# ami-iit/paper_gorbani_2025_humanoids_multi-rate-mpc-ironcub

Hardware: AMD Instinct MI355X
Metric: MPC solves/sec (whole node) + p50 single-solve latency, iRonCub paper horizon (higher is better)
Workload: dtype f64

## Files before the change

paper_gorbani_2025_humanoids_multi-rate-mpc-ironcub_amd/csrc/vsmpc_solve_body.inc:

```
#define VS_STAMP(i)                                                                        \
    do {                                                                                    \
        if constexpr (STAMPS) {                                                             \
            unsigned long long* st_ = late_args()->stamps;                                  \
            if (tid == 0 && st_ != nullptr) st_[size_t(blockIdx.x) * 16 + (i)] = __builtin_amdgcn_s_memtime(); \
        }                                                                                   \
    } while (0)
    unsigned long long t_acc[6] = {0, 0, 0, 0, 0, 0};
    unsigned long long t_mark = 0, stamp_t1 = 0, rt0 = 0;
    if constexpr (STAMPS) rt0 = __builtin_amdgcn_s_memrealtime();
#define VS_TIC()                                                     \
    do {                                                             \
        if constexpr (STAMPS) t_mark = __builtin_amdgcn_s_memtime(); \
    } while (0)
#define VS_TOC(i)                                                          \
    do {                                                                   \
        if constexpr (STAMPS) {                                            \
            const unsigned long long t_now = __builtin_amdgcn_s_memtime(); \
            t_acc[i] += t_now - t_mark;                                    \
            t_mark = t_now;                                                \
        }                                                                  \
    } while (0)
    using S = Smem<D, SMALL>;
    static_assert(!SMALL || (FORM == 1 && !TUNED), "the small-batch kind is the structured form of the shared kind");
    constexpr bool PIPE = FORM == 1;
    constexpr int QR_P0_STEPS = D::STRUCT_LONG ? 1 : 2;
    extern __shared__ __attribute__((aligned(16))) double smem[];
    double* sIn = smem + S::oIn;
    double* sA = smem + S::oA;
    double* sBj = smem + S::oBj;
    double* sBt = smem + S::oBt;
    double* sC = smem + S::oC;
    double* sVprev = smem + S::oVprev;
    double* sInvD = smem + S::oInvD;
    double* sW = smem + S::oW;
    double* sZ = smem + S::oZ;
    double* sSv = smem + S::oSv;
    double* sSvec = smem + S::oSvec;
    double* sV = smem + S::oV;
    double* sX = smem + S::oX;
    double* sF = smem + S::oF;
    double* sDt = smem + S::oDt;
    double* sCfg = smem + S::oCfg;
    int* sFlags = reinterpret_cast<int*>(smem + S::oFlags);
    double* sY = smem + S::oY;
    double* Lb = smem + S::oM;
    double* sXinv = smem + S::oXinv;
    double* sQP = smem + S::oQP;
    double* sU = smem + S::oU;

    const int inst = blockIdx.x;
    if (inst >= batch) return;
    int tid = threadIdx.x;
    int lane = tid & 63;
    const int wave = __builtin_amdgcn_readfirstlane(tid >> 6);
#define VS_REFRESH_IDS()                                                                     \
    do {                                                                                     \
        unsigned m_ = ~0u;                                                                   \
        asm volatile("" : "+s"(m_));                                                         \
        lane = int(__builtin_amdgcn_mbcnt_hi(m_, __builtin_amdgcn_mbcnt_lo(m_, 0u)));        \
        tid = (wave << 6) | lane;                                                            \
    } while (0)

    constexpr int TPW = TileTab<D, PIPE>::TPW;

    VS_STAMP(0);
    {
        static_assert(D::NIN % 2 == 0 && D::NVAR % 2 == 0 && D::NXS % 2 == 0 && D::NUO % 2 == 0, "double2 I/O");
        static_assert(D::NIN / 2 <= D::BLOCK, "one 16-byte load per thread covers the record");
        const double2* in2 = reinterpret_cast<const double2*>(in + size_t(inst) * D::NIN);
        double2* sIn2 = reinterpret_cast<double2*>(sIn);
        double2 rec = make_double2(0.0, 0.0);
        if (tid < D::NIN / 2) rec = in2[tid];
        constexpr int TUN0 = D::BLOCK - CFG_SIZE / 2;
        double2 trow = make_double2(0.0, 0.0);
        if constexpr (TUNED) {
            static_assert(CFG_SIZE == VSMPC_TUNE_SIZE && CFG_SIZE % 2 == 0 && CFG_VMAX == CFG_SIZE - 2, "row = sCfg + one pad");
            if (tid >= TUN0) trow = reinterpret_cast<const double2*>(tun + size_t(inst) * CFG_SIZE)[tid - TUN0];
        }
        if (tid < 4) sFlags[tid] = 0;
        if (tid < D::N) sDt[tid] = cfg.dt[tid];
        if constexpr (!TUNED) {
            if (tid >= 64 && tid < 64 + NWROWS) sCfg[CFG_SQ + tid - 64] = cfg.sq[tid - 64];
            if (tid >= 96 && tid < 96 + NJ) sCfg[CFG_WJ + tid - 96] = cfg.wj[tid - 96];
            if (tid == 128) {
                sCfg[CFG_WREG] = cfg.w_reg; sCfg[CFG_WTHR] = cfg.w_thr; sCfg[CFG_WINIT] = cfg.w_init;
                sCfg[CFG_VMIN] = cfg.vmin; sCfg[CFG_VMAX] = cfg.vmax;
            }
        }
        for (int i = tid; i < NX * NX + NX * NJ + NX * NTH + 28; i += D::BLOCK) sA[i] = 0.0;
        if (tid < D::NIN / 2) sIn2[tid] = rec;
        if constexpr (TUNED) {
            if (tid >= TUN0) {
                sCfg[2 * (tid - TUN0)] = trow.x;
                sCfg[2 * (tid - TUN0) + 1] = trow.y;
            }
            const bool fin = isfinite(trow.x) && (isfinite(trow.y) || tid == D::BLOCK - 1);
            __syncthreads();
            if (!fin) sFlags[0] = 1;
        } else {
            __syncthreads();
        }
    }
    p0_linearize<false, false, false>(cfg.use_jet, sIn, sA, sBj, sBt, sC, sVprev, tid, D::BLOCK);
    if (wave == 3) {
        if constexpr (FORM == 1) p0_joint_reduction<D, 0, QR_P0_STEPS>(smem, lane);
        else p0_joint_reduction<D>(smem, lane);
    }

    constexpr int NJROW = D::NV + NTH + 1, ZROW = D::NV + NTH;
    double* sJetT = sXinv;
    if constexpr (SMALL) sJetT = smem + S::oJetT;
    static_assert(SMALL || S::oJetT == S::oXinv, "the jet trajectories lie at the head of the X region");
    double* sGA = sJetT + NJROW * D::N;
    static_assert(D::NV + NTH <= 64 && (SMALL || NJROW * D::N + 6 * D::N <= S::NXT * D::TS), "jet trajectories fit the X region");
    if (wave == 1) {
        if (lane < D::NV + NTH) {
            const bool affl = lane >= D::NV;
            const int i = affl ? lane - D::NV : (lane & 3);
            const int blk = affl ? -1 : v_block_of_internal<D>(lane);
            const double jon = sA[(12 + i) * NX + 16 + i], ja = sA[(16 + i) * NX + 12 + i], jb = sA[(16 + i) * NX + 16 + i];
            const double c12 = sC[12 + i], c16 = sC[16 + i], b12 = sBt[(12 + i) * NTH + i], b16 = sBt[(16 + i) * NTH + i];
            const double t0 = sIn[VSMPC_IN_X0 + 12 + i], td0 = sIn[VSMPC_IN_X0 + 16 + i];
            const double bT = affl ? c12 : b12, bTd = affl ? c16 : b16;
            double T = affl ? t0 : 0.0, Td = affl ? td0 : 0.0;
#pragma unroll
            for (int k = 0; k < D::N; ++k) {
                sJetT[lane * D::N + k] = T;
                const double mT = (affl || throttle_block_of_stage<D>(k) == blk) ? 1.0 : 0.0;
                const double dT = fma(jon, Td, mT * bT);
                const double dTd = fma(ja, T, fma(jb, Td, mT * bTd));
                const double dt = sDt[k];
                T = fma(dt, dT, T);
                Td = fma(dt, dTd, Td);
            }
        }
        for (int k = lane; k < D::N; k += 64) sJetT[ZROW * D::N + k] = 0.0;
        if constexpr (FORM == 1) {
            const double am = sIn[VSMPC_IN_ALPHA] * sIn[VSMPC_IN_MASS];
            const double* R = sIn + VSMPC_IN_WRB;
            const double* gr = sIn + VSMPC_IN_GRAV;
            for (int e = lane; e < 6 * D::N; e += 64) {
                const int h = e / (3 * D::N), k = (e / 3) % D::N, r = e % 3;
                double g = 0.0;
#pragma unroll
                for (int c = 0; c < NTH; ++c) g = fma(sIn[VSMPC_IN_AMOM + (3 * h + r) * NTH + c], sJetT[(D::NV + c) * D::N + k], g);
                const double ch = h == 0 ? am * (R[0 + r] * gr[0] + R[3 + r] * gr[1] + R[6 + r] * gr[2]) : 0.0;
                sGA[e] = g + ch;
            }
        }
    }
    if constexpr (FORM == 1) {
        if (wave == 2) {
            for (int e = lane; e < S::sizeZero; e += 64) smem[S::oSZero + e] = 0.0;
            for (int e = lane; e < 12 * D::NREF; e += 64) {
                const int row = e % 12;
                const double off = row < 3 ? -sIn[VSMPC_IN_PREF + row] : ((row >= 6 && row < 9) ? -sIn[VSMPC_IN_RPYINIT + row - 6] : 0.0);
                smem[S::oSRefC + e] = sIn[VSMPC_IN_XREF + e] + off;
            }
        }
    }
    if constexpr (FORM == 1 && D::STRUCT_LONG) {
        for (int e = tid; e < S::sizeAc; e += D::BLOCK) smem[S::oSAc + e] = 0.0;
    }
    __syncthreads();
    if constexpr (FORM != 1) {
        for (int e = tid; e < 6 * D::N; e += D::BLOCK) {
            const int h = e / (3 * D::N), k = (e / 3) % D::N, r = e % 3, row = (h ? 9 : 3) + r;
            double g = 0.0;
#pragma unroll
            for (int c = 0; c < NTH; ++c) g = fma(sA[row * NX + 12 + c], sJetT[(D::NV + c) * D::N + k], g);
            sGA[e] = g;
        }
        __syncthreads();
    }

    VS_STAMP(1);
    VS_REFRESH_IDS();
    if constexpr (STAMPS) stamp_t1 = __builtin_amdgcn_s_memtime();
    d4 acc[TPW];
    if constexpr (FORM == 1) {
        static_assert(D::STRUCT_P1, "structured condensing is instantiated for horizons with Dims::STRUCT_P1");
        VS_TIC();
        if (wave < 2) {
            p1s_chain<D, 0, SMALL>(cfg, wave, lane, smem);
            if (wave == 0) p0_joint_reduction<D, QR_P0_STEPS, NJC>(smem, lane);
        } else {
            p1s_chain<D, 1, SMALL>(cfg, wave - 2, lane, smem);
        }
        VS_TOC(0);
        __syncthreads();
        VS_TOC(1);
        if constexpr (!D::STRUCT_LONG) {
            p1s_contract<D, SMALL>(smem, tid);
            __syncthreads();
        }
        VS_TOC(3);
        auto tail = [&](auto wcst) __attribute__((always_inline)) {
            constexpr int W = decltype(wcst)::value;
            if constexpr (SMALL) {
                static_for<0, TPW>([&](auto qcst) __attribute__((always_inline)) {
                    constexpr int q = decltype(qcst)::value;
                    if constexpr (small_instalment<D, TPW, W>(q) < 0) acc[q] = d4{0.0, 0.0, 0.0, 0.0};
                });
                const int ln0 = fresh_lane();
                small_form<D, TPW, W, 0>(sCfg, acc, Lb, smem + S::oQR + S::QR_GY, sVprev, ln0, (ln0 >> 4) * 17 + (ln0 & 15));
            } else {
                p1s_entries<D, TPW, W, PIPE>(acc, smem, lane);
            }
            VS_TOC(2);
            __syncthreads();
            VS_STAMP(2);
            constexpr TileTab<D, PIPE> tab{};
            double* dbgLw = nullptr;
            if constexpr (STAMPS && !SMALL) {
                double* dbgM = late_args()->dbgM;
                double* dbgL = late_args()->dbgL;
                dbgLw = dbgL != nullptr ? dbgL + size_t(inst) * D::NP * D::NP : nullptr;
                if (dbgM != nullptr) {
                    const int ln = fresh_lane();
                    static_for<0, TPW>([&](auto qcst) __attribute__((always_inline)) {
                        constexpr int q = decltype(qcst)::value;
                        constexpr int t = q * D::NWAVES + W;
                        if constexpr (tab.forms(t, W))
                            dump_hessian_tile<D>(dbgM + size_t(inst) * D::NP * D::NP, tab.ti[t], tab.tj[t], acc[q], sCfg,
                                                 smem + S::oQR + S::QR_GY, sVprev, ln);
                    });
                }
            }
            VS_STAMP(3);
            if constexpr (D::WG_PER_CU == 1) pin_tiles_agpr<TPW>(acc);
            const int ln = fresh_lane();
            cholesky_wave<D, TPW, W, STAMPS, PIPE, SMALL>(sCfg, acc, Lb, sInvD, smem + S::oQR + S::QR_GY, sVprev, sFlags, sXinv, sW, dbgLw, ln,
                                                  (ln >> 4) * 17 + (ln & 15), (ln & 15) * 17 + (ln >> 4), sZ);
            if constexpr (STAMPS) {
                if (dbgLw != nullptr) {
                    const int l2 = fresh_lane();
                    static_for<0, TPW>([&](auto qcst) __attribute__((always_inline)) {
                        constexpr int q = decltype(qcst)::value;
                        constexpr int t = q * D::NWAVES + W;
                        if constexpr (tab.holds(t, W) && tab.tj[t] < D::PVT && tab.ti[t] > tab.tj[t])
                            dump_factor_tile<D>(dbgLw, tab.ti[t], tab.tj[t], acc[q], l2);
                    });
                }
            }
        };
        switch (wave) {
            case 0: tail(std::integral_constant<int, 0>{}); break;
            case 1: tail(std::integral_constant<int, 1>{}); break;
            case 2: tail(std::integral_constant<int, 2>{}); break;
            default: tail(std::integral_constant<int, 3>{}); break;
        }
    } else {
#pragma unroll
        for (int q = 0; q < TPW; ++q) acc[q] = d4{0.0, 0.0, 0.0, 0.0};
        constexpr int CPT = D::CPT;
        const int pw = wave;
        const int ptid = tid;
        const int half = pw / (D::NWAVES / 2);
        const int xr0 = half ? 6 : 0, hr0 = half ? 9 : 3, er0 = half ? 23 : 20;
        const int yx0 = half ? 6 : 0, yh0 = half ? 9 : 3, ye0 = half ? 15 : 12;

        double M1[9], Sk[9], Ce[3], sqx[3], sqh[3], sqe[3];
        auto load_coeffs = [&]() __attribute__((always_inline)) {
#pragma unroll
            for (int r = 0; r < 3; ++r) {
#pragma unroll
                for (int c = 0; c < 3; ++c) {
                    M1[3 * r + c] = sA[(xr0 + r) * NX + hr0 + c];
                    Sk[3 * r + c] = sA[(hr0 + r) * NX + hr0 + c];
                }
                Ce[r] = sC[er0 + r];
                sqx[r] = sCfg[CFG_SQ + yx0 + r];
                sqh[r] = sCfg[CFG_SQ + yh0 + r];
                sqe[r] = sCfg[CFG_SQ + ye0 + r];
            }
        };
        const int ylane = (lane >> 4) * D::YS + (lane & 15);
        constexpr int NPASS = (D::N + 1) / 2;
        if constexpr (STAMPS) { t_mark = stamp_t1; VS_TOC(3); }

        int col[CPT], kind[CPT], blk[CPT];
        double aff[CPT], xs[CPT][3], hs[CPT][3], es[CPT][3], bha[CPT][3];
        const double* jetT[CPT];
        const double* gaT = sGA + half * 3 * D::N;
#pragma unroll
        for (int cc = 0; cc < CPT; ++cc) {
            const int c = cc * D::PCOLS + ptid % D::PCOLS;
            int comp = 0;
            col[cc] = c;
            kind[cc] = 3;
            blk[cc] = 0;
            if (c < D::NUY) { kind[cc] = 0; blk[cc] = c / NJC; comp = c - NJC * blk[cc]; }
            else if (c >= D::NU && c < D::NZ) { kind[cc] = 1; blk[cc] = v_block_of_internal<D>(c - D::NU); comp = (c - D::NU) & 3; }
            else if (c == D::NZ) { kind[cc] = 2; }
            const int jc = comp & 7, tc = comp & 3;
            const bool aff_col = kind[cc] == 2, jnt_col = kind[cc] == 0, thr_col = kind[cc] == 1;
            aff[cc] = aff_col ? 1.0 : 0.0;
#pragma unroll
            for (int r = 0; r < 3; ++r) {
                const double x0 = sIn[VSMPC_IN_X0 + xr0 + r], h0 = sIn[VSMPC_IN_X0 + hr0 + r], e0 = sIn[VSMPC_IN_X0 + er0 + r];
                const double bj = sBj[(hr0 + r) * NJ + jc], ch = sC[hr0 + r], at = sA[(hr0 + r) * NX + 12 + tc];
                xs[cc][r] = aff_col ? x0 : 0.0;
                hs[cc][r] = aff_col ? h0 : 0.0;
                es[cc][r] = aff_col ? e0 : 0.0;
                bha[cc][r] = jnt_col ? bj : (aff_col ? ch : (thr_col ? at : 0.0));
            }
            jetT[cc] = sJetT + (thr_col ? c - D::NU : ZROW) * D::N;
        }
        unsigned tpk[TilePack<D>::NWORDS];
#pragma unroll
        for (int k = 0; k < TilePack<D>::NWORDS; ++k) tpk[k] = kTilePack<D>.w[pw][k];
        const double* ybase = sY + ylane;
        constexpr bool UNROLLED = TPW <= SYRK_UNROLL_TPW;
        auto slot_word = [&](int q) __attribute__((always_inline)) {
            unsigned w = tpk[q >> 1];
            if constexpr (!UNROLLED) asm volatile("" : "+s"(w));
            return w;
        };
        auto slot_a = [&](int q) __attribute__((always_inline)) { return ybase + 16 * int((slot_word(q) >> (16 * (q & 1))) & 0xffu); };
        auto slot_b = [&](int q) __attribute__((always_inline)) { return ybase + 16 * int((slot_word(q) >> (16 * (q & 1) + 8)) & 0xffu); };
        auto rec_pass = [&](int m, int nnodes, double* sYm) __attribute__((always_inline)) {
            load_coeffs();
#pragma unroll
            for (int par = 0; par < 2; ++par) {
                if (par >= nnodes) break;
                const int k = 2 * m + par;
                const double dt = sDt[k];
                const int rc = k < D::NS ? 0 : k - D::NS;
                const double* xr = sIn + VSMPC_IN_XREF + rc * 12;
                double xrx[3], xrh[3], ga[3];
#pragma unroll
                for (int r = 0; r < 3; ++r) { xrx[r] = xr[yx0 + r]; xrh[r] = xr[yh0 + r]; ga[r] = gaT[3 * k + r]; }
#pragma unroll
                for (int cc = 0; cc < CPT; ++cc) {
                    const double tk = jetT[cc][k];
                    const bool actJ = (kind[cc] == 0 && joint_block_of_stage<D>(k) == blk[cc]) || kind[cc] == 2;
                    const double scale = kind[cc] == 1 ? tk : (actJ ? 1.0 : 0.0);
                    double dx[3], dh[3], de[3];
#pragma unroll
                    for (int r = 0; r < 3; ++r) {
                        double a0 = M1[3 * r] * hs[cc][0], a1 = scale * bha[cc][r], a2 = aff[cc] * ga[r];
#pragma unroll
                        for (int c = 1; c < 3; ++c) a0 = fma(M1[3 * r + c], hs[cc][c], a0);
#pragma unroll
                        for (int c = 0; c < 3; ++c) a1 = fma(Sk[3 * r + c], hs[cc][c], a1);
                        dx[r] = a0;
                        dh[r] = a1 + a2;
                        de[r] = fma(aff[cc], Ce[r], xs[cc][r]);
                    }
#pragma unroll
                    for (int r = 0; r < 3; ++r) { xs[cc][r] += dt * dx[r]; hs[cc][r] += dt * dh[r]; es[cc][r] += dt * de[r]; }
                    if (CPT == 1 || col[cc] < D::NP) {
                        double* Yn = sYm + 18 * par * D::YS + col[cc];
#pragma unroll
                        for (int r = 0; r < 3; ++r) {
                            const double vx = fma(-aff[cc], xrx[r], xs[cc][r]);
                            const double vh = fma(-aff[cc], xrh[r], hs[cc][r]);
                            Yn[(yx0 + r) * D::YS] = sqx[r] * vx;
                            Yn[(yh0 + r) * D::YS] = sqh[r] * vh;
                            Yn[(ye0 + r) * D::YS] = sqe[r] * es[cc][r];
                        }
                    }
                }
            }
            if (nnodes == 1)
                for (int i = ptid; i < 2 * D::YS; i += D::BLOCK) sYm[18 * D::YS + i] = 0.0;
        };
        auto syrk_fixed = [&](auto nks_c, auto nact_c) __attribute__((always_inline)) {
            constexpr int NKS = decltype(nks_c)::value, NACT = decltype(nact_c)::value;
            if constexpr (NACT > 0) {
                double ha[SYRK_DIST], hb[SYRK_DIST];
#pragma unroll
                for (int ks = 0; ks < SYRK_DIST; ++ks) {
                    ha[ks] = slot_a(NACT - 1)[ks * 4 * D::YS];
                    hb[ks] = slot_b(NACT - 1)[ks * 4 * D::YS];
                }
#pragma unroll
                for (int q = NACT - 1; q >= 0; --q) {
                    const int qn = q > 0 ? q - 1 : 0;
                    syrk_slot<D, NKS, true>(acc[q], slot_a(q), slot_b(q), ha, hb, slot_a(qn), slot_b(qn));
                }
            }
        };
        if constexpr (UNROLLED) {
            static_for<0, NPASS>([&](auto mc) __attribute__((always_inline)) {
                constexpr int m = decltype(mc)::value;
                constexpr int nnodes = (2 * m + 1 < D::N) ? 2 : 1;
                VS_TIC();
                rec_pass(m, nnodes, sY);
                VS_TOC(0);
                __syncthreads();
                VS_TOC(1);
                syrk_fixed(std::integral_constant<int, nnodes == 2 ? 9 : 5>{}, std::integral_constant<int, nact_max<D>(m)>{});
                VS_TOC(2);
                __syncthreads();
            });
        } else {
            static_for<0, PassGroups<D>::count()>([&](auto gc) __attribute__((always_inline)) {
                constexpr PassGroups<D> pg{};
                constexpr int g = decltype(gc)::value;
#pragma unroll 1
                for (int m = pg.start[g]; m < pg.end[g]; ++m) {
                    VS_TIC();
                    rec_pass(m, pg.nks[g] == 9 ? 2 : 1, sY);
                    VS_TOC(0);
                    __syncthreads();
                    VS_TOC(1);
                    syrk_fixed(std::integral_constant<int, pg.nks[g]>{}, std::integral_constant<int, pg.nact[g]>{});
                    VS_TOC(2);
                    __syncthreads();
                }
            });
        }
        VS_TIC();
    }
    VS_REFRESH_IDS();
    if constexpr (D::WG_PER_CU == 1) pin_tiles_agpr<TPW>(acc);

    static_assert(D::NWAVES == 4, "wave-specialised phases are instantiated for four wavefronts");
    constexpr int PVT = D::PVT;
    const int crow = (lane >> 4) * 17 + (lane & 15);
    const int lrow = (lane & 15) * 17 + (lane >> 4);
    double* dbgL = STAMPS ? late_args()->dbgL : nullptr;
    double* dbgLi = dbgL != nullptr ? dbgL + size_t(inst) * D::NP * D::NP : nullptr;
    VS_REFRESH_IDS();
    if constexpr (!PIPE) {
        int wave_c = wave;
        if constexpr (STAMPS) asm volatile("" : "+s"(wave_c));
        VS_STAMP(2);
        if constexpr (STAMPS) {
            const TileTab<D, PIPE>& tab = kTileTab<D, PIPE>;
            double* dbgM = late_args()->dbgM;
            if (dbgM != nullptr) {
#pragma unroll
                for (int q = 0; q < TPW; ++q) {
                    const int t = q * D::NWAVES + wave, tc = q * D::NWAVES + wave_c;
                    if (tab.forms(t, wave))
                        dump_hessian_tile<D>(dbgM + size_t(inst) * D::NP * D::NP, tab.ti[tc], tab.tj[tc], acc[q], sCfg,
                                             smem + S::oQR + S::QR_GY, sVprev, lane);
                }
            }
        }
        VS_STAMP(3);
        switch (wave) {
            case 0: cholesky_wave<D, TPW, 0, STAMPS, PIPE>(sCfg, acc, Lb, sInvD, smem + S::oQR + S::QR_GY, sVprev, sFlags, sXinv, sW, dbgLi, lane, crow, lrow, sZ); break;
            case 1: cholesky_wave<D, TPW, 1, STAMPS, PIPE>(sCfg, acc, Lb, sInvD, smem + S::oQR + S::QR_GY, sVprev, sFlags, sXinv, sW, dbgLi, lane, crow, lrow, sZ); break;
            case 2: cholesky_wave<D, TPW, 2, STAMPS, PIPE>(sCfg, acc, Lb, sInvD, smem + S::oQR + S::QR_GY, sVprev, sFlags, sXinv, sW, dbgLi, lane, crow, lrow, sZ); break;
            default: cholesky_wave<D, TPW, 3, STAMPS, PIPE>(sCfg, acc, Lb, sInvD, smem + S::oQR + S::QR_GY, sVprev, sFlags, sXinv, sW, dbgLi, lane, crow, lrow, sZ); break;
        }
        if constexpr (STAMPS) {
            const TileTab<D, PIPE>& tab = kTileTab<D, PIPE>;
            if (dbgLi != nullptr) {
#pragma unroll
                for (int q = 0; q < TPW; ++q) {
                    const int t = q * D::NWAVES + wave, tc = q * D::NWAVES + wave_c;
                    if (tab.holds(t, wave) && tab.tj[tc] < PVT && tab.ti[tc] > tab.tj[tc])
                        dump_factor_tile<D>(dbgLi, tab.ti[tc], tab.tj[tc], acc[q], lane);
                }
            }
        }
    }
    if (STAMPS && dbgLi != nullptr) {
        for (int e = tid; e < (D::NP - 16 * PVT) * (D::NP - 16 * PVT); e += D::BLOCK) {
            const int gr = 16 * PVT + e / (D::NP - 16 * PVT), gc = 16 * PVT + e % (D::NP - 16 * PVT);
            if (gc <= gr) dbgLi[size_t(gr) * D::NP + gc] = Lb[lower_at<D>(gr, gc)];
        }
    }

    VS_STAMP(4);
    VS_REFRESH_IDS();
    if constexpr (D::WG_PER_CU == 1) pin_tiles_agpr<TPW>(acc);
    const bool hold = sIn[VSMPC_IN_HOLD] != 0.0;
    constexpr int PV = D::PVT;
    auto init_corner_rhs = [&]() {
        if (tid >= 16 * PV && tid < D::NP) sW[tid] = tid < D::NZ ? -Lb[lower_at<D>(D::NZ, tid)] : 0.0;
    };
    init_corner_rhs();
    if (tid < D::NP) sZ[tid] = (hold && tid >= D::NZ - 4 && tid < D::NZ) ? sVprev[tid - (D::NZ - 4)] : 0.0;
    __syncthreads();

    auto corner_update = [&](int p) __attribute__((always_inline)) {
        if (p > PV) {
            if (tid >= 16 * PV && tid < 16 * p) {
                const double* T = Lb + tile_off<D>(p, tid >> 4) + (tid & 15);
                const double* zp = sZ + 16 * p;
                double a2 = 0.0;
#pragma unroll
                for (int k = 0; k < 16; ++k) a2 += T[k * 17] * zp[k];
                sW[tid] -= a2;
            }
            __syncthreads();
        }
    };
    auto sweep_tile = [&](int p, bool prescribed) {
        if (wave == 0) {
            const int j = lane & 15;
            const int gj = 16 * p + j;
            const double* Tpp = Lb + tile_off<D>(p, p) + j;
            double colv[16];
#pragma unroll
            for (int k = 0; k < 16; ++k) {
                const double t = Tpp[k * 17];
                colv[k] = k >= j ? t : 0.0;
            }
            double w = sW[gj];
            const bool fix = (gj >= D::NZ) || (gj >= D::NU && (prescribed || (hold && gj >= D::NZ - 4)));
            const double inv_eff = fix ? 0.0 : sInvD[gj];
            const double zadd = (fix && gj < D::NZ) ? sZ[gj] : 0.0;
            double z = 0.0;
#pragma unroll
            for (int k = 15; k >= 0; --k) {
                const double zk = readlane_f64(fma(w, inv_eff, zadd), k);
                z = (j == k) ? zk : z;
                w = fma(-colv[k], zk, w);
            }
            if (lane < 16) sZ[gj] = z;
        }
        __syncthreads();
        corner_update(p);
    };

    constexpr bool DUALQP = S::DUALQP;
    if constexpr (DUALQP) {
        constexpr int PL = D::NT - 1, KL = D::NZ - 16 * PL;
        static_assert(KL == D::NV - 16 && KL >= 4, "pins live in the last tile row");
        const double* X6 = sXinv + PV * D::TS;
        const double* L76 = Lb + tile_off<D>(PL, PV);
        const double* L77 = Lb + tile_off<D>(PL, PL);
        if (wave == 0) {
            const int j = lane & 15;
            const int gj = 16 * PL + j;
            const double* Tpp = L77 + j;
            double colv[KL], l76[KL], x6[16];
#pragma unroll
            for (int k = 0; k < KL; ++k) {
                const double t = Tpp[k * 17];
                colv[k] = k >= j ? t : 0.0;
                l76[k] = L76[k * 17 + j];
            }
#pragma unroll
            for (int i = 0; i < 16; ++i) x6[i] = X6[i * 17 + j];
            double w = sW[gj];
            double w6 = sW[16 * PV + j];
            const bool fix = (j >= KL) || (hold && j >= KL - 4);
            const double inv_eff = fix ? 0.0 : sInvD[gj];
            const double zadd = (fix && j < KL) ? sZ[gj] : 0.0;
            double z = 0.0;
#pragma unroll
            for (int k = KL - 1; k >= 0; --k) {
                const double zk = readlane_f64(fma(w, inv_eff, zadd), k);
                z = (j == k) ? zk : z;
                w = fma(-colv[k], zk, w);
                w6 = fma(-l76[k], zk, w6);
            }
            double z6 = 0.0;
#pragma unroll
            for (int i = 0; i < 16; ++i) z6 = fma(x6[i], readlane_f64(w6, i), z6);
            if (lane < 16) { sZ[gj] = z; sZ[16 * PV + j] = z6; }
        } else {
            dual_setup_beside_sweep<D>(wave, lane);
        }
    } else if constexpr (S::DUAL3) {
        static_assert(D::NT - 1 == PV + 2, "three throttle tile rows");
        double x2[16];
        const double* L22d = Lb + tile_off_c<D>(PV + 2, PV + 2);
        const double* inv2 = sInvD + D::NU + 32;
        if (wave == 1) tile_inverse_rows<0, 8>(L22d, inv2, x2, lane);
        sweep_tile(PV + 2, false);
        auto sweep_tile_x = [&](int p, const double* Xp) {
            if (wave == 0) {
                const int j = lane & 15;
                double z0 = 0.0, z1 = 0.0;
#pragma unroll
                for (int k = 0; k < 16; k += 2) {
                    z0 = fma(Xp[k * 17 + j], sW[16 * p + k], z0);
                    z1 = fma(Xp[(k + 1) * 17 + j], sW[16 * p + k + 1], z1);
                }
                if (lane < 16) sZ[16 * p + j] = z0 + z1;
            }
            __syncthreads();
            corner_update(p);
        };
        if (wave == 1) tile_inverse_rows<8, 13>(L22d, inv2, x2, lane);
        sweep_tile_x(PV + 1, smem + S::oDual3T0);
        if (wave == 1) {
            tile_inverse_rows<13, 16>(L22d, inv2, x2, lane);
            if (lane < 16) {
#pragma unroll
                for (int i = 0; i < 16; ++i) smem[S::oDual3T1 + i * 17 + lane] = x2[i];
            }
        }
        sweep_tile_x(PV, sXinv + PV * D::TS);
    } else {
#pragma unroll 1
        for (int p = D::NT - 1; p >= PV; --p) sweep_tile(p, false);
    }
    if (wave == 0) {
        const bool valid = lane < D::NV;
        const double v = sZ[D::NU + (valid ? lane : 0)];
        const bool fixed = hold && lane >= D::NV - 4;
        const double tolv = 1e-12 * (1.0 + fabs(v));
        const bool viol = valid && !fixed && (v < sCfg[CFG_VMIN] - tolv || v > sCfg[CFG_VMAX] + tolv);
        const unsigned long long vm = __ballot(viol);
        if (lane == 0) { sFlags[3] = __popcll(vm); sFlags[1] = VSMPC_STATUS_SOLVED; sFlags[2] = 1; }
        if constexpr (DUALQP) {
            if (lane == 0) sFlags[4] = int(unsigned(vm));
        }
    }
    __syncthreads();
    const bool need_qp = sFlags[3] != 0;
    VS_STAMP(5);
    VS_REFRESH_IDS();

#ifdef VS_DIAG_QP
    for (int i = 0; i < 4; ++i) t_acc[i] = 0;
    unsigned long long* const qp_cycles = STAMPS ? t_acc : nullptr;
#else
    constexpr unsigned long long* qp_cycles = nullptr;
#endif
    if (need_qp) {
        box_qp<D>(sFlags[3], hold, wave, qp_cycles);
        __syncthreads();
        VS_STAMP(6);
        VS_REFRESH_IDS();
        if constexpr (D::NU % 16 != 0) {
            init_corner_rhs();
            __syncthreads();
#pragma unroll 1
            for (int p = D::NT - 1; p >= PV; --p) sweep_tile(p, true);
        }
    } else {
        VS_STAMP(6);
    }
    switch (wave) {
        case 0:
            if constexpr (PIPE) p5_wave0_jets<D>(smem, lane);
            else backsub_wave<D, TPW, 0, PIPE>(acc, sW, sZ, sXinv, sU, lane);
            break;
        case 1: backsub_wave<D, TPW, 1, PIPE>(acc, sW, sZ, sXinv, sU, lane); break;
        case 2: backsub_wave<D, TPW, 2, PIPE>(acc, sW, sZ, sXinv, sU, lane); break;
        default: backsub_wave<D, TPW, 3, PIPE>(acc, sW, sZ, sXinv, sU, lane); break;
    }
    if (tid < D::NV) sV[tid] = sZ[D::NU + tid];
    __syncthreads();

    VS_STAMP(7);
    VS_REFRESH_IDS();
#ifdef VS_DIAG_P6
    for (int i = 0; i < 4; ++i) t_acc[i] = 0;
    VS_TIC();
#define VS_P6_TOC(i) VS_TOC(i)
#else
#define VS_P6_TOC(i) do { } while (0)
#endif
    const SolveArgs* ka = late_args();
    double* xout = ka->xout;
    double* fmout = ka->fmout;
    int* status_out = ka->status_out;
    int* iters_out = ka->iters_out;
    auto write_first_move = [&](int l) __attribute__((always_inline)) {
        double v;
        if (l < 8) v = sU[l];
        else if (l < 12) v = sV[D::NV - 4 + (l - 8)];
        else if (l < 16) v = Jet::throttle_of_v(sV[D::NV - 4 + (l - 12)]);
        else if (l < 20) v = sX[NX + 12 + (l - 16)];
        else v = sX[NX + 16 + (l - 20)];
        fmout[size_t(inst) * VSMPC_FM_SIZE + l] = v;
    };
    double u8[8] = {0.0, 0.0, 0.0, 0.0, 0.0, 0.0, 0.0, 0.0};
    constexpr int JX_SPLIT = PIPE ? 3 : NJC;
    if (PIPE && wave == 3 && lane < D::HC) joint_expand<D, NJC, JX_SPLIT>(smem + S::oQR, sZ + NJC * lane, u8);
    {
        constexpr int ROWS = PIPE ? 6 : NX;
        constexpr int NE = ROWS * D::N, RND = (NE + D::BLOCK - 1) / D::BLOCK;
#pragma unroll
        for (int rd = 0; rd < RND; ++rd) {
            const int e0 = tid + rd * D::BLOCK, ec = e0 < NE ? e0 : NE - 1;
            const int k = ec / ROWS, rr = ec - k * ROWS;
            const int r = PIPE ? (rr < 3 ? 3 + rr : 6 + rr) : rr;
            const int e = NX * k + r;
            const int jb = joint_block_of_stage<D>(k);
            const int tb = throttle_block_of_stage<D>(k);
            const int vq = tb == 0 ? D::NV - 4 : 4 * (tb - 1);
            double f = sC[r];
#pragma unroll
            for (int c = 0; c < NJC; ++c) f += sBj[r * NJ + c] * sZ[NJC * jb + c];
#pragma unroll
            for (int c = 0; c < NTH; ++c) f += sBt[r * NTH + c] * sV[vq + c];
            if (e0 < NE) sF[e] = f;
        }
    }
    __syncthreads();
    VS_P6_TOC(0);
    {
        constexpr int CHK = D::N > 20 ? 9 : 6, NCH = (D::N + CHK - 1) / CHK;
        double jT = 0.0, jTd = 0.0, jon = 0.0, ja = 0.0, jb = 0.0;
        double Sk[9], hh[3] = {0.0, 0.0, 0.0};
        double cm0 = 0.0, cm1 = 0.0, cm2 = 0.0, cce = 0.0, cx = 0.0, cee = 0.0;
        const int hr0m = (lane & 1) ? 9 : 3;
        const int cg = lane / 3, cr = lane - 3 * cg;
        const int cxr = (cg ? 6 : 0) + cr, chr0 = cg ? 9 : 3, cer = (cg ? 23 : 20) + cr;
        constexpr int JOFF = PIPE ? 0 : 1;
        if (!PIPE && wave == 0 && lane < NTH) {
            jon = sA[(12 + lane) * NX + 16 + lane]; ja = sA[(16 + lane) * NX + 12 + lane]; jb = sA[(16 + lane) * NX + 16 + lane];
            jT = sIn[VSMPC_IN_X0 + 12 + lane]; jTd = sIn[VSMPC_IN_X0 + 16 + lane];
            sX[12 + lane] = jT;
            sX[16 + lane] = jTd;
        }
        if (wave == 1 && lane < 2) {
#pragma unroll
            for (int r = 0; r < 3; ++r) {
                hh[r] = sIn[VSMPC_IN_X0 + hr0m + r];
                sX[hr0m + r] = hh[r];
#pragma unroll
                for (int c = 0; c < 3; ++c) Sk[3 * r + c] = sA[(hr0m + r) * NX + hr0m + c];
            }
        }
        if (wave == 2 && lane < 6) {
            cm0 = sA[cxr * NX + chr0]; cm1 = sA[cxr * NX + chr0 + 1]; cm2 = sA[cxr * NX + chr0 + 2];
            cce = sC[cer];
            cx = sIn[VSMPC_IN_X0 + cxr]; cee = sIn[VSMPC_IN_X0 + cer];
            sX[cxr] = cx;
            sX[cer] = cee;
        }
        static_assert(D::NUO <= D::NWAVES * D::NP, "joint increments fit the partial-sum array");
        if (wave == 3 && lane < D::HC) {
            if constexpr (PIPE) joint_expand<D, JX_SPLIT, 0>(smem + S::oQR, sZ + NJC * lane, u8);
            else joint_expand<D>(smem + S::oQR, sZ + NJC * lane, u8);
#pragma unroll
            for (int i = 0; i < 8; ++i) sU[NJ * lane + i] = u8[i];
        }
        if (wave == 3 && xout != nullptr) {
            double2* xo = reinterpret_cast<double2*>(xout + size_t(inst) * D::NVAR);
            for (int i = lane; i < D::NUO / 2; i += 64) xo[D::NXS / 2 + i] = make_double2(sU[2 * i], sU[2 * i + 1]);
            if (lane < D::NV / 2) {
                const int e = 2 * lane, b = e >> 2, c = e & 3;
                const int q = b == 0 ? D::NV - 4 + c : 4 * (b - 1) + c;
                xo[(D::NXS + D::NUO) / 2 + lane] = make_double2(sV[q], sV[q + 1]);
            }
        }

        static_for<0, NCH + 1 + JOFF>([&](auto scst) __attribute__((always_inline)) {
            constexpr int st = decltype(scst)::value;
            if constexpr (!PIPE && st < NCH) {
                if (wave == 0 && lane < NTH) {
                    constexpr int k0 = st * CHK;
                    double fa[CHK], fb[CHK], dtk[CHK];
#pragma unroll
                    for (int u = 0; u < CHK; ++u) {
                        const int k = (k0 + u < D::N) ? k0 + u : D::N - 1;
                        fa[u] = sF[NX * k + 12 + lane];
                        fb[u] = sF[NX * k + 16 + lane];
                        dtk[u] = sDt[k];
                    }
#pragma unroll
                    for (int u = 0; u < CHK; ++u) {
                        const double dT = fma(jon, jTd, fa[u]);
                        const double dTd = fma(ja, jT, fma(jb, jTd, fb[u]));
                        jT = fma(dtk[u], dT, jT);
                        jTd = fma(dtk[u], dTd, jTd);
                        if (k0 + u < D::N) {
                            sX[NX * (k0 + u + 1) + 12 + lane] = jT;
                            sX[NX * (k0 + u + 1) + 16 + lane] = jTd;
                        }
                    }
                }
            }
            if constexpr (PIPE && st == 1) {
                if (wave == 3 && fmout != nullptr && lane < VSMPC_FM_SIZE) write_first_move(lane);
            }
            if constexpr (st >= JOFF && st - JOFF < NCH) {
                if (wave == 1) {
                    constexpr int k0 = (st - JOFF) * CHK;
                    constexpr int kn = k0 + CHK < D::N ? CHK : D::N - k0;
                    if (lane < 6 * kn) {
                        const int k = k0 + lane / 6, rr = lane % 6, row = rr < 3 ? 3 + rr : 6 + rr;
                        double gk = sF[NX * k + row];
#pragma unroll
                        for (int c = 0; c < NTH; ++c) gk = fma(sA[row * NX + 12 + c], sX[NX * k + 12 + c], gk);
                        sF[NX * k + row] = gk;
                    }
                    if (lane < 2) {
                        double gk[CHK][3], dtk[CHK];
#pragma unroll
                        for (int u = 0; u < CHK; ++u) {
                            const int k = (k0 + u < D::N) ? k0 + u : D::N - 1;
#pragma unroll
                            for (int r = 0; r < 3; ++r) gk[u][r] = sF[NX * k + hr0m + r];
                            dtk[u] = sDt[k];
                        }
#pragma unroll
                        for (int u = 0; u < CHK; ++u) {
                            double dh[3];
#pragma unroll
                            for (int r = 0; r < 3; ++r)
                                dh[r] = fma(Sk[3 * r], hh[0], fma(Sk[3 * r + 1], hh[1], fma(Sk[3 * r + 2], hh[2], gk[u][r])));
#pragma unroll
                            for (int r = 0; r < 3; ++r) hh[r] = fma(dtk[u], dh[r], hh[r]);
                            if (k0 + u < D::N) {
#pragma unroll
                                for (int r = 0; r < 3; ++r) sX[NX * (k0 + u + 1) + hr0m + r] = hh[r];
                            }
                        }
                    }
                }
            }
            if constexpr (st >= JOFF + 1 && st - JOFF - 1 < NCH) {
                if (wave == 2 && lane < 6) {
                    constexpr int k0 = (st - JOFF - 1) * CHK;
                    double hk[CHK][3], dtk[CHK];
#pragma unroll
                    for (int u = 0; u < CHK; ++u) {
                        const int k = (k0 + u < D::N) ? k0 + u : D::N - 1;
#pragma unroll
                        for (int c = 0; c < 3; ++c) hk[u][c] = sX[NX * k + chr0 + c];
                        dtk[u] = sDt[k];
                    }
#pragma unroll
                    for (int u = 0; u < CHK; ++u) {
                        const double dx = fma(cm0, hk[u][0], fma(cm1, hk[u][1], cm2 * hk[u][2]));
                        cee = fma(dtk[u], cx + cce, cee);
                        cx = fma(dtk[u], dx, cx);
                        if (k0 + u < D::N) {
                            sX[NX * (k0 + u + 1) + cxr] = cx;
                            sX[NX * (k0 + u + 1) + cer] = cee;
                        }
                    }
                }
            }
            if constexpr (st + 1 < NCH + 1 + JOFF) __syncthreads();
            if constexpr (st == 0) VS_P6_TOC(1);
        });
    }
    __syncthreads();
    VS_P6_TOC(2);
    VS_STAMP(8);
    VS_REFRESH_IDS();

    if (xout != nullptr) {
        double2* xo = reinterpret_cast<double2*>(xout + size_t(inst) * D::NVAR);
        for (int i = tid; i < D::NXS / 2; i += D::BLOCK) xo[i] = make_double2(sX[2 * i], sX[2 * i + 1]);
    }
    if (!PIPE && fmout != nullptr && tid < VSMPC_FM_SIZE) write_first_move(tid);
    if (tid == 0) {
        int st = sFlags[1];
        if (sFlags[0]) st = VSMPC_STATUS_NUMERICAL;
        status_out[inst] = st;
        if (iters_out != nullptr) iters_out[inst] = sFlags[2];
    }
    VS_P6_TOC(3);
    VS_STAMP(9);
    if constexpr (STAMPS) {
        unsigned long long* st_ = late_args()->stamps;
        if (tid == 0 && st_ != nullptr) {
#if defined(VS_DIAG_P3) && !defined(VS_DIAG_P6)
            for (int i = 0; i < 4; ++i) t_acc[i] = vs_diag_p3[i];
#endif
            t_acc[5] = __builtin_amdgcn_s_memrealtime() - rt0;
            t_acc[4] = rt0;
            for (int i = 0; i < 6; ++i) st_[size_t(blockIdx.x) * 16 + 10 + i] = t_acc[i];
        }
    }
#undef VS_STAMP
#undef VS_REFRESH_IDS
#undef VS_TIC
#undef VS_TOC
#undef VS_P6_TOC
```

Measured before the change: 8.138 million.

## Replace chunked multi-barrier state rollout with single-wave DPP recurrence in pipelined form

In the pipelined form, the throttle-coupling term is folded into the forcing pass, and the chunked rollout with a barrier per chunk is replaced by one wave that integrates momentum and position rows. That wave uses DPP broadcast FMAs in inline asm to exchange the 3x3 coupling across lanes, with no block-wide syncs. The remaining output writes (joint expansion, xout, first move) are spread across the other waves so they overlap with the recurrence. This removes several __syncthreads and serial chunk handoffs, but relies on hand-written asm, hazard nops and scratch stores into spare shared memory, which raises the correctness risk. It also changes VS_P6_TOC(2) so it only runs when the diagnostic macro is defined.

```diff
diff --git a/paper_gorbani_2025_humanoids_multi-rate-mpc-ironcub_amd/csrc/vsmpc_solve_body.inc b/paper_gorbani_2025_humanoids_multi-rate-mpc-ironcub_amd/csrc/vsmpc_solve_body.inc
--- a/paper_gorbani_2025_humanoids_multi-rate-mpc-ironcub_amd/csrc/vsmpc_solve_body.inc
+++ b/paper_gorbani_2025_humanoids_multi-rate-mpc-ironcub_amd/csrc/vsmpc_solve_body.inc
@@ -671,13 +671,14 @@
     constexpr int JX_SPLIT = PIPE ? 3 : NJC;
     if (PIPE && wave == 3 && lane < D::HC) joint_expand<D, NJC, JX_SPLIT>(smem + S::oQR, sZ + NJC * lane, u8);
     {
-        constexpr int ROWS = PIPE ? 6 : NX;
+        constexpr int ROWS = PIPE ? 7 : NX;
         constexpr int NE = ROWS * D::N, RND = (NE + D::BLOCK - 1) / D::BLOCK;
+        static_assert(!PIPE || RND == 1, "the forcing of the pipelined schedule is one round");
 #pragma unroll
         for (int rd = 0; rd < RND; ++rd) {
             const int e0 = tid + rd * D::BLOCK, ec = e0 < NE ? e0 : NE - 1;
             const int k = ec / ROWS, rr = ec - k * ROWS;
-            const int r = PIPE ? (rr < 3 ? 3 + rr : 6 + rr) : rr;
+            const int r = PIPE ? (rr < 3 ? 3 + rr : (rr < 6 ? 6 + rr : 0)) : rr;
             const int e = NX * k + r;
             const int jb = joint_block_of_stage<D>(k);
             const int tb = throttle_block_of_stage<D>(k);
@@ -687,12 +688,17 @@
             for (int c = 0; c < NJC; ++c) f += sBj[r * NJ + c] * sZ[NJC * jb + c];
 #pragma unroll
             for (int c = 0; c < NTH; ++c) f += sBt[r * NTH + c] * sV[vq + c];
+            if constexpr (PIPE) {
+#pragma unroll
+                for (int c = 0; c < NTH; ++c) f = fma(sA[r * NX + 12 + c], sX[NX * k + 12 + c], f);
+                if (rr == 6) f = -0.0;
+            }
             if (e0 < NE) sF[e] = f;
         }
     }
     __syncthreads();
     VS_P6_TOC(0);
-    {
+    if constexpr (!PIPE) {
         constexpr int CHK = D::N > 20 ? 9 : 6, NCH = (D::N + CHK - 1) / CHK;
         double jT = 0.0, jTd = 0.0, jon = 0.0, ja = 0.0, jb = 0.0;
         double Sk[9], hh[3] = {0.0, 0.0, 0.0};
@@ -700,8 +706,8 @@
         const int hr0m = (lane & 1) ? 9 : 3;
         const int cg = lane / 3, cr = lane - 3 * cg;
         const int cxr = (cg ? 6 : 0) + cr, chr0 = cg ? 9 : 3, cer = (cg ? 23 : 20) + cr;
-        constexpr int JOFF = PIPE ? 0 : 1;
-        if (!PIPE && wave == 0 && lane < NTH) {
+        constexpr int JOFF = 1;
+        if (wave == 0 && lane < NTH) {
             jon = sA[(12 + lane) * NX + 16 + lane]; ja = sA[(16 + lane) * NX + 12 + lane]; jb = sA[(16 + lane) * NX + 16 + lane];
             jT = sIn[VSMPC_IN_X0 + 12 + lane]; jTd = sIn[VSMPC_IN_X0 + 16 + lane];
             sX[12 + lane] = jT;
@@ -725,8 +731,7 @@
         }
         static_assert(D::NUO <= D::NWAVES * D::NP, "joint increments fit the partial-sum array");
         if (wave == 3 && lane < D::HC) {
-            if constexpr (PIPE) joint_expand<D, JX_SPLIT, 0>(smem + S::oQR, sZ + NJC * lane, u8);
-            else joint_expand<D>(smem + S::oQR, sZ + NJC * lane, u8);
+            joint_expand<D>(smem + S::oQR, sZ + NJC * lane, u8);
 #pragma unroll
             for (int i = 0; i < 8; ++i) sU[NJ * lane + i] = u8[i];
         }
@@ -742,7 +747,7 @@
 
         static_for<0, NCH + 1 + JOFF>([&](auto scst) __attribute__((always_inline)) {
             constexpr int st = decltype(scst)::value;
-            if constexpr (!PIPE && st < NCH) {
+            if constexpr (st < NCH) {
                 if (wave == 0 && lane < NTH) {
                     constexpr int k0 = st * CHK;
                     double fa[CHK], fb[CHK], dtk[CHK];
@@ -766,9 +771,6 @@
                     }
                 }
             }
-            if constexpr (PIPE && st == 1) {
-                if (wave == 3 && fmout != nullptr && lane < VSMPC_FM_SIZE) write_first_move(lane);
-            }
             if constexpr (st >= JOFF && st - JOFF < NCH) {
                 if (wave == 1) {
                     constexpr int k0 = (st - JOFF) * CHK;
@@ -831,9 +833,97 @@
             if constexpr (st + 1 < NCH + 1 + JOFF) __syncthreads();
             if constexpr (st == 0) VS_P6_TOC(1);
         });
+    } else {
+        constexpr int JUNK = 128 + NX * (D::N + 1);
+        static_assert(JUNK + 2 <= S::NXT * D::TS, "the ownerless stores of the stream stay inside the X region");
+        double* junk = sXinv;
+#ifdef VS_DIAG_P6
+        unsigned long long* p6t = reinterpret_cast<unsigned long long*>(junk + JUNK);
+#endif
+        if (wave == 1) {
+#ifdef VS_DIAG_P6
+            if constexpr (STAMPS) { if (lane == 0) p6t[0] = __builtin_amdgcn_s_memtime(); }
+#endif
+            const int half = (lane >> 4) & 1, l = lane & 15;
+            const bool own = lane < 32 && l < 6, mom = own && l < 3, integ = own && !mom;
+            const int r3 = l < 3 ? l : (l < 6 ? l - 3 : 0);
+            const int hc0 = half ? 9 : 3;
+            const int srow = (l < 3 ? hc0 : (half ? 6 : 0)) + r3, cer = (half ? 23 : 20) + r3;
+            double c0 = sA[srow * NX + hc0], c1 = sA[srow * NX + hc0 + 1], c2 = sA[srow * NX + hc0 + 2];
+            double cce = sC[cer], xs = sIn[VSMPC_IN_X0 + srow], ee = sIn[VSMPC_IN_X0 + cer];
+            c0 = own ? c0 : 0.0; c1 = own ? c1 : 0.0; c2 = own ? c2 : 0.0;
+            xs = own ? xs : 0.0;
+            cce = integ ? cce : 0.0;
+            ee = integ ? ee : 0.0;
+            double* xp = own ? sX + srow : junk + lane;
+            double* ep = integ ? sX + cer : junk + 64 + lane;
+            const double* gp = sF + (mom ? srow : 0);
+            xp[0] = xs;
+            ep[0] = ee;
+            constexpr int NSB = (D::N + 23) / 24, CHS = (D::N + NSB - 1) / NSB;
+#pragma unroll
+            for (int sb = 0; sb < NSB; ++sb) {
+                double gk[CHS], dtk[CHS];
+#pragma unroll
+                for (int u = 0; u < CHS; ++u) {
+                    const int k = (sb * CHS + u < D::N) ? sb * CHS + u : D::N - 1;
+                    gk[u] = gp[NX * k];
+                    dtk[u] = sDt[k];
+                }
+#pragma unroll
+                for (int u = 0; u < CHS; ++u) {
+                    const int k = sb * CHS + u;
+                    if (k < D::N) {
+                        if (k == 0)
+                            asm volatile("s_nop 4\n\tv_fmac_f64_dpp %0, %1, %2 row_newbcast:2 row_mask:0xf bank_mask:0xf" : "+v"(gk[u]) : "v"(xs), "v"(c2));
+                        else
+                            asm volatile("s_nop 1\n\tv_fmac_f64_dpp %0, %1, %2 row_newbcast:2 row_mask:0xf bank_mask:0xf" : "+v"(gk[u]) : "v"(xs), "v"(c2));
+                        asm volatile("v_fmac_f64_dpp %0, %1, %2 row_newbcast:1 row_mask:0xf bank_mask:0xf" : "+v"(gk[u]) : "v"(xs), "v"(c1));
+                        asm volatile("v_fmac_f64_dpp %0, %1, %2 row_newbcast:0 row_mask:0xf bank_mask:0xf" : "+v"(gk[u]) : "v"(xs), "v"(c0));
+                        ee = fma(dtk[u], xs + cce, ee);
+                        xs = fma(dtk[u], gk[u], xs);
+                        xp[NX * (k + 1)] = xs;
+                        ep[NX * (k + 1)] = ee;
+                    }
+                }
+            }
+#ifdef VS_DIAG_P6
+            if constexpr (STAMPS) { if (lane == 0) p6t[1] = __builtin_amdgcn_s_memtime(); }
+#endif
+        }
+        static_assert(D::NUO <= D::NWAVES * D::NP, "joint increments fit the partial-sum array");
+        if (wave == 3) {
+            if (lane < D::HC) {
+                joint_expand<D, JX_SPLIT, 0>(smem + S::oQR, sZ + NJC * lane, u8);
+#pragma unroll
+                for (int i = 0; i < 8; ++i) sU[NJ * lane + i] = u8[i];
+            }
+            if (xout != nullptr) {
+                double2* xo = reinterpret_cast<double2*>(xout + size_t(inst) * D::NVAR);
+                for (int i = lane; i < D::NUO / 2; i += 64) xo[D::NXS / 2 + i] = make_double2(sU[2 * i], sU[2 * i + 1]);
+            }
+            if (fmout != nullptr && lane < 8) write_first_move(lane);
+        }
+        if (wave == 0 && xout != nullptr && lane < D::NV / 2) {
+            double2* xo = reinterpret_cast<double2*>(xout + size_t(inst) * D::NVAR);
+            const int e = 2 * lane, b = e >> 2, c = e & 3;
+            const int q = b == 0 ? D::NV - 4 + c : 4 * (b - 1) + c;
+            xo[(D::NXS + D::NUO) / 2 + lane] = make_double2(sV[q], sV[q + 1]);
+        }
+        if (wave == 2 && fmout != nullptr && lane < VSMPC_FM_SIZE - 8) write_first_move(8 + lane);
     }
     __syncthreads();
-    VS_P6_TOC(2);
+#ifdef VS_DIAG_P6
+    if constexpr (STAMPS && PIPE) {
+        const unsigned long long* p6t = reinterpret_cast<const unsigned long long*>(sXinv + 128 + NX * (D::N + 1));
+        const unsigned long long t_now = __builtin_amdgcn_s_memtime();
+        t_acc[1] = p6t[1] - p6t[0];
+        t_acc[2] = t_now - p6t[1];
+        t_mark = t_now;
+    } else {
+        VS_P6_TOC(2);
+    }
+#endif
     VS_STAMP(8);
     VS_REFRESH_IDS();
 
```

Result: faster. 8.466 million (median of 6 runs) (+4.0%).
